# sunshinnnn/DSMnet

Hardware: AMD Instinct MI355X
Metric: stereo pairs/sec forward, PSMNet D=192 384×1280, at 1/2/4/8 MI355X (higher is better)
Workload: dtype f32

## Files before the change

dsmnet_amd/_lib.py:

```python
import ctypes
import os

_HERE = os.path.dirname(os.path.abspath(__file__))
LIB_PATH = os.environ.get("DSM_LIB_PATH") or os.path.join(_HERE, "csrc", "libdsmnet_hip.so")

c_int, c_void_p, c_size_t = ctypes.c_int, ctypes.c_void_p, ctypes.c_size_t

DSM_OK = 0
DSM_F32 = 0
DSM_NCDHW, DSM_NDHWC = 0, 1
DSM_CONV_FP32_MFMA, DSM_CONV_COUT1_CHUNKED, DSM_CONV_TM_SHIFT, DSM_CONV_BLOCKS_SHIFT = 1, 2, 4, 16
DSM_CONV_NO_NSPLIT = 4
DSM_CONV_NO_ONCE = 8
DSM_CONV_KSPLIT_SHIFT = 8
DSM_PREC_F32, DSM_PREC_F16, DSM_PREC_F16X2 = 0, 1, 2


class Bn3dArgs(ctypes.Structure):
    _fields_ = [("y", c_void_p), ("residual", c_void_p), ("out", c_void_p), ("gamma", c_void_p),
                ("beta", c_void_p), ("running_mean", c_void_p), ("running_var", c_void_p),
                ("affine", c_void_p), ("workspace", c_void_p), ("gout", c_void_p), ("dy", c_void_p),
                ("dresidual", c_void_p), ("B", c_int), ("C", c_int),
                ("Dy", c_int), ("Hy", c_int), ("Wy", c_int), ("Dr", c_int), ("Hr", c_int), ("Wr", c_int),
                ("relu", c_int), ("momentum", ctypes.c_float), ("eps", ctypes.c_float),
# ... 42 lines not shown
class ColorRecord(ctypes.Structure):
    _fields_ = [("order", c_int * 4), ("jitter", ctypes.c_float * 4), ("flags", c_int), ("alpha_row", c_int)]


DSM_COLOR_JITTER, DSM_COLOR_LIGHTING, DSM_COLOR_NORMALIZE = 1, 2, 4
DSM_COLOR_MAX_RECORDS = 64


SIGNATURES = {
    "dsm_abi_version": (c_int, []),
    "dsm_strerror": (ctypes.c_char_p, [c_int]),
    "dsm_corr1d_fwd": (c_int, [c_void_p] * 4 + [c_int] * 8 + [c_void_p]),
    "dsm_corr1d_bwd": (c_int, [c_void_p] * 6 + [c_int] * 8 + [c_void_p]),
    "dsm_concat_volume_fwd": (c_int, [c_void_p] * 3 + [c_int] * 8 + [c_void_p]),
    "dsm_concat_volume_bwd": (c_int, [c_void_p] * 3 + [c_int] * 8 + [c_void_p]),
    "dsm_soft_argmin_fwd": (c_int, [c_void_p] * 3 + [c_int] * 10 + [c_void_p]),
    "dsm_soft_argmin_bwd": (c_int, [c_void_p] * 5 + [c_int] * 10 + [c_void_p]),
    "dsm_corr1d_plan": (c_int, [c_void_p] * 4 + [c_int] * 8 + [ctypes.c_char_p, c_int]),
    "dsm_concat_volume_fwd_plan": (c_int, [c_void_p] * 3 + [c_int] * 8 + [ctypes.c_char_p, c_int]),
    "dsm_concat_volume_bwd_plan": (c_int, [c_void_p] * 3 + [c_int] * 8 + [ctypes.c_char_p, c_int]),
    "dsm_soft_argmin_fwd_plan": (c_int, [c_void_p] * 3 + [c_int] * 10 + [ctypes.c_char_p, c_int]),
    "dsm_soft_argmin_bwd_plan": (c_int, [c_void_p] * 5 + [c_int] * 10 + [ctypes.c_char_p, c_int]),
    "dsm_conv3d_packed_weight_bytes": (c_size_t, [c_int] * 3),
    "dsm_conv3d_pack_weights": (c_int, [c_void_p] * 2 + [c_int] * 3 + [c_void_p]),
    "dsm_conv_pack_weights": (c_int, [c_void_p] * 2 + [c_int] * 5 + [c_void_p]),
    "dsm_absmax": (c_int, [c_void_p, c_size_t, c_void_p, c_void_p]),
    "dsm_conv3d_fwd": (c_int, [ctypes.POINTER(Conv3dArgs), c_void_p]),
    "dsm_basicblock2d_fwd": (c_int, [ctypes.POINTER(BasicBlock2dArgs), c_void_p]),
    "dsm_conv3d_plan": (c_int, [ctypes.POINTER(Conv3dArgs), ctypes.c_char_p, c_int]),
    "dsm_conv3d_workspace_bytes": (c_size_t, [ctypes.POINTER(Conv3dArgs)]),
    "dsm_conv3d_wgrad": (c_int, [c_void_p] * 4 + [c_int] * 12 + [c_void_p] * 3),
    "dsm_conv2d_wgrad": (c_int, [c_void_p] * 4 + [c_int] * 11 + [c_void_p] * 3),
    "dsm_conv3d_cout1_bwd": (c_int, [c_void_p] * 5 + [c_int] * 5 + [c_void_p]),
    "dsm_deconv3d_cout1_bwd": (c_int, [c_void_p] * 5 + [c_int] * 8 + [c_void_p]),
    "dsm_bn3d_train_fwd": (c_int, [ctypes.POINTER(Bn3dArgs), c_void_p]),
    "dsm_bn3d_train_bwd": (c_int, [ctypes.POINTER(Bn3dArgs), c_void_p]),
    "dsm_decoder_cat": (c_int, [c_void_p] * 5 + [c_int] * 11 + [c_void_p]),
    "dsm_stage_images_nhwc16": (c_int, [c_void_p] * 3 + [c_int] * 4 + [c_void_p]),
    "dsm_volume_relayout": (c_int, [c_void_p] * 2 + [c_int] * 6 + [c_void_p]),
    "dsm_conv_packed_weight_bytes": (ctypes.c_size_t, [c_int] * 4),
    "dsm_spp_branch_floats": (ctypes.c_size_t, [c_int] * 3),
    "dsm_spp_pool8": (c_int, [c_void_p] * 2 + [c_int] * 3 + [c_void_p]),
    "dsm_spp_branches": (c_int, [c_void_p] * 5 + [c_int] * 3 + [c_void_p]),
    "dsm_spp_concat": (c_int, [c_void_p] * 4 + [c_int] * 3 + [c_void_p] * 2),
    "dsm_warp_abs_error": (c_int, [c_void_p] * 4 + [c_int] * 6 + [ctypes.c_float, c_void_p]),
    "dsm_selfsup_workspace_floats": (c_size_t, [ctypes.POINTER(SelfsupItem), c_int]),
    "dsm_selfsup_fwd": (c_int, [ctypes.POINTER(SelfsupItem), c_int, c_int] + [c_void_p] * 4),
    "dsm_selfsup_bwd": (c_int, [ctypes.POINTER(SelfsupItem), c_int, c_int] + [c_void_p] * 4),
    "dsm_suploss_workspace_floats": (c_size_t, [c_int] * 5),
    "dsm_suploss_fwd": (c_int, [ctypes.POINTER(SuplossItem), c_int, c_void_p, c_int, c_int, c_int, c_int] + [c_void_p] * 4),
    "dsm_suploss_bwd": (c_int, [ctypes.POINTER(SuplossItem), c_int, c_void_p, c_int, c_int, c_int] + [c_void_p] * 4),
    "dsm_stereo_color": (c_int, [c_void_p, c_void_p, ctypes.POINTER(ColorRecord)] + [c_int] * 6 + [c_void_p]),
    "dsm_concat_conv_fwd": (c_int, [c_void_p] * 5 + [c_size_t] + [c_void_p] * 2 + [c_int] * 9 + [c_void_p]),
}

_lib = None


class DsmnetHipError(RuntimeError):
    pass


def _bind_torch_hip_runtime():
    import torch
    hip = os.path.join(os.path.dirname(torch.__file__), "lib", "libamdhip64.so")
    if os.path.exists(hip):
        ctypes.CDLL(hip, mode=ctypes.RTLD_GLOBAL)


def load():
    global _lib
    if _lib is not None:
        return _lib
    if not os.path.exists(LIB_PATH):
        raise DsmnetHipError(
            "libdsmnet_hip.so not found at %s -- build it with "
            "`python -m dsmnet_amd.csrc.build` (there is no CPU fallback)" % LIB_PATH)
    _bind_torch_hip_runtime()
    lib = ctypes.CDLL(LIB_PATH)
    for name, (res, args) in SIGNATURES.items():
        fn = getattr(lib, name)
        fn.restype = res
        fn.argtypes = args
    if lib.dsm_abi_version() != 7:
        raise DsmnetHipError("libdsmnet_hip.so ABI version mismatch")
    _lib = lib
    return lib


def check(code, what):
    if code != DSM_OK:
        msg = load().dsm_strerror(code).decode()
        raise DsmnetHipError("%s failed: %s (code %d)" % (what, msg, code))
```

dsmnet_amd/blocks2d.py:

```python
import torch
import torch.nn as nn
import torch.nn.functional as F

from . import costvolume as cv
from . import blocks3d
from .blocks3d import _versions

_TRAIN_2D_MODE = __import__("os").environ.get("DSM_TRAIN_2D", "auto")
_FUSED_TRAIN_2D = _TRAIN_2D_MODE in ("auto", "fused", "conv")
_FUSED_TRAIN_2D_BN = _TRAIN_2D_MODE == "fused"
_TRAIN_2D_MIN_PIXELS = int(__import__("os").environ.get("DSM_TRAIN_2D_MIN_PIXELS", 65536)) if _TRAIN_2D_MODE == "auto" else 0


class own_kernels_only(object):

    def __enter__(self):
        global _TRAIN_2D_MIN_PIXELS, _FUSED_TRAIN_2D
        self.saved = (_TRAIN_2D_MIN_PIXELS, _FUSED_TRAIN_2D)
        _TRAIN_2D_MIN_PIXELS, _FUSED_TRAIN_2D = 0, True
        return self

    def __exit__(self, *exc):
        global _TRAIN_2D_MIN_PIXELS, _FUSED_TRAIN_2D
        _TRAIN_2D_MIN_PIXELS, _FUSED_TRAIN_2D = self.saved
        return False


def fused_ok(conv, x):
    if not (isinstance(conv, nn.Conv2d) and x.is_cuda and x.dtype == torch.float32):
        return False
    k, s, d, p = conv.kernel_size, conv.stride, conv.dilation, conv.padding
    if k[0] != k[1] or s[0] != s[1] or d[0] != d[1] or p[0] != p[1] or conv.groups != 1:
        return False
    if k[0] not in (1, 3) or s[0] not in (1, 2) or d[0] not in (1, 2):
        return False
    if p[0] != d[0] * (k[0] - 1) // 2 or conv.padding_mode != "zeros":
        return False
    if conv.out_channels in cv.WIDE2D_COUT:
        return _wide_ok(conv, x)
    if conv.out_channels not in (32, 64, 128):
        return False
    cin = x.shape[1]
    if cin % 16 != 0 or cin < conv.in_channels:
        return False
    return cv.conv2d_variant(conv.out_channels, s[0], k[0], d[0])


_WIDE2D_EXCLUDED = frozenset()


def _wide_ok(conv, x):
    if conv.kernel_size[0] != 3 or conv.dilation[0] != 1 or cv.get_option("conv_precision") not in ("f16x2", "f16"):
        return False
    B, cin, H, W = x.shape
    s = conv.stride[0]
    if cin % 16 != 0 or cin != conv.in_channels or (cin, conv.out_channels, s) in _WIDE2D_EXCLUDED:
        return False
    Ho, Wo = (H - 1) // s + 1, (W - 1) // s + 1
    if Wo > (2032 if s == 1 else 1016) or B * Ho * Wo >= 2 ** 20:
        return False
    return 4 * B * cin * H * W < 2 ** 31 and B * Ho * Wo * conv.out_channels < 2 ** 31 - 1


class _Folded2d(object):
    def __init__(self):
        self.key = None
        self.packed = self.scale = self.shift = None

    def get(self, conv, bn, cin_padded):
        srcs = [conv.weight, conv.bias]
        if bn is not None:
            srcs += [bn.weight, bn.bias, bn.running_mean, bn.running_var]
        key = _versions(*srcs) + (cin_padded,)
        if key != self.key:
            with torch.no_grad():
                self.packed = cv.pack_conv2d_weight(conv.weight, cin_padded)
                if bn is not None:
                    inv = torch.rsqrt(bn.running_var + bn.eps)
                    scale = bn.weight * inv if bn.weight is not None else inv
                    shift = -bn.running_mean * scale
                    if bn.bias is not None:
                        shift = shift + bn.bias
                    if conv.bias is not None:
                        shift = shift + conv.bias * scale
                    self.scale, self.shift = scale.contiguous(), shift.contiguous()
                elif conv.bias is not None:
                    self.scale = torch.ones_like(conv.bias)
                    self.shift = conv.bias.detach().clone()
                else:
                    self.scale = self.shift = None
            self.key = key
        return self.packed, self.scale, self.shift


def train_ok(conv, x):
    if not (_FUSED_TRAIN_2D and isinstance(conv, nn.Conv2d) and torch.is_tensor(x) and x.is_cuda and
            x.dtype == torch.float32 and conv.weight.dtype == torch.float32):
        return False
    k, s, d, p = conv.kernel_size, conv.stride, conv.dilation, conv.padding
    if k[0] != k[1] or s[0] != s[1] or d[0] != d[1] or p[0] != p[1] or conv.groups != 1:
        return False
    if conv.bias is not None or conv.padding_mode != "zeros" or p[0] != d[0] * (k[0] // 2):
        return False
    if x.shape[0] * ((x.shape[2] - 1) // s[0] + 1) * ((x.shape[3] - 1) // s[0] + 1) < _TRAIN_2D_MIN_PIXELS:
        return False
    return x.shape[1] == conv.in_channels and cv.conv2d_variant(conv.out_channels, s[0], k[0], d[0])


def _run_conv2d_autograd(conv, bn, x, residual, relu):
    y = cv.conv2d(x, conv.weight, conv.stride[0], conv.dilation[0])
    if (bn is not None and bn.training and _FUSED_TRAIN_2D_BN and blocks3d._FUSED_TRAIN_BN and
            y.shape[1] % 4 == 0 and y.shape[1] <= 256):
        momentum = bn.momentum if bn.momentum is not None else 0.1
        out = cv.bn_add_relu2d(y, bn.weight, bn.bias, residual,
                               bn.running_mean if bn.track_running_stats else None,
                               bn.running_var if bn.track_running_stats else None,
                               1 if relu else 0, momentum, bn.eps)
        if bn.num_batches_tracked is not None:
            bn.num_batches_tracked += 1
        blocks3d._bump_running_stats(bn)
        return out
    if bn is not None:
        y = bn(y)
    if residual is not None:
        y = y + residual
    return F.relu(y) if relu else y


def run_conv2d(folded, conv, bn, x, residual=None, relu=False):
    training = bn is not None and bn.training
    if not training and not torch.is_grad_enabled() and fused_ok(conv, x):
        packed, scale, shift = folded.get(conv, bn, x.shape[1])
        return cv.conv2d_block(x, packed, conv.out_channels, scale, shift, residual,
                               stride=conv.stride[0], relu=1 if relu else 0,
                               k=conv.kernel_size[0], dilation=conv.dilation[0])
    if train_ok(conv, x):
        return _run_conv2d_autograd(conv, bn, x, residual, relu)
    if x.shape[1] != conv.in_channels:
        x = x[:, : conv.in_channels]
    y = conv(x)
    if bn is not None:
        y = bn(y)
    if residual is not None:
        y = y + residual
    return F.relu(y) if relu else y


def run_basicblock_layers(fold1, c1, b1, fold2, c2, b2, x, relu_after, skip=True):
    if b1 is None or b2 is None or c1.training or b1.training or b2.training or torch.is_grad_enabled():
        return None
    if not (fused_ok(c1, x) and fused_ok(c2, x) and c1.kernel_size[0] == 3 and c2.kernel_size[0] == 3 and
            c2.stride[0] == 1 and c2.dilation[0] == 1 and c2.in_channels == c2.out_channels == c1.out_channels and
            cv.basicblock2d_ok(x, c1.in_channels, c1.out_channels, c1.stride[0], c1.dilation[0])):
        return None
    p1, s1, h1 = fold1.get(c1, b1, x.shape[1])
    p2, s2, h2 = fold2.get(c2, b2, x.shape[1])
    return cv.basicblock2d(x, p1, s1, h1, p2, s2, h2, relu=relu_after, skip=skip)


def run_basicblock(cb1, cb2, x, downsample):
    if downsample is not None or not isinstance(cb1, ConvBN2d) or not isinstance(cb2, ConvBN2d):
        return None
    return run_basicblock_layers(cb1._folded, cb1[0], cb1[1], cb2._folded, cb2[0], cb2[1], x, False)


class ConvBN2d(nn.Sequential):

    def __init__(self, conv, bn):
        super(ConvBN2d, self).__init__(conv, bn)
        self._folded = _Folded2d()

    def forward(self, x, residual=None, relu=False):
        return run_conv2d(self._folded, self[0], self[1], x, residual, relu)


def stage_image_nhwc16(img):
    return cv.stage_images_nhwc16(img, None)
```

dsmnet_amd/costvolume.py:

```python
import ctypes

import torch

from . import _lib

_CL3D = torch.channels_last_3d


class LaunchTimer(object):

    def __init__(self):
        self.records = []

    def start(self):
        ev = torch.cuda.Event(enable_timing=True)
        ev.record()
        return ev

    def stop(self, name, start, work):
        ev = torch.cuda.Event(enable_timing=True)
        ev.record()
        self.records.append((name, start, ev, work))

    def summary(self):
# ... 313 lines not shown
    a.x = x.data_ptr()
    a.w_packed = packed_weight.data_ptr()
    a.y = y.data_ptr()
    a.scale = None if scale is None else scale.data_ptr()
    a.shift = None if shift is None else shift.data_ptr()
    a.residual = None if residual is None else residual.data_ptr()
    a.B, a.Cin, a.Cout = B, cin, cout
    a.Di, a.Hi, a.Wi = Di, Hi, Wi
    a.Do, a.Ho, a.Wo = Do, Ho, Wo
    a.stride, a.transposed, a.relu = int(stride), int(transposed), int(relu)
    a.flags = _conv_flags()
    if virtual is not None:
        a.vol_virtual, a.vol_mask_left = 1, int(virtual.mask_left)
    keep = _set_precision(a, x, y if cout > 1 else None)
    vox = B * (Di * Hi * Wi if transposed else Do * Ho * Wo)
    work = 54.0 * cin * cout * vox if cout > 1 else 4.0 * B * (cin * Di * Hi * Wi + Do * Ho * Wo)
    with torch.cuda.device(x.device), _timed(lambda: conv3d_plan_name(a), work):
        rc = _lib.load().dsm_conv3d_fwd(ctypes.byref(a), _stream())
    _lib.check(rc, "dsm_conv3d_fwd")
    del keep
    return y


def conv3d_plan_name(args):
    buf = ctypes.create_string_buffer(96)
    _lib.check(_lib.load().dsm_conv3d_plan(ctypes.byref(args), buf, 96), "dsm_conv3d_plan")
    return buf.value.decode()


import os as _os

_PRECISIONS = ("bf16x3", "fp32", "f16x2", "f16")


def _env_precision():
    v = _os.environ.get("DSM_CONV_PRECISION", "")
    if v and v not in _PRECISIONS:
        raise ValueError("DSM_CONV_PRECISION must be one of %s, got %r" % (_PRECISIONS, v))
    return v or "f16x2"


def _env_flag(name, default):
    v = _os.environ.get(name, "")
    if v not in ("", "0", "1"):
        raise ValueError("%s must be 0 or 1, got %r" % (name, v))
    return default if v == "" else v == "1"


_WIDE_CONV2D_DEFAULT = False

_OPTIONS = {"fuse_volume": True, "fuse_blocks": True, "conv_precision": _env_precision(), "conv_flags": 0,
            "separable_volume": _env_flag("DSM_SEPARABLE_VOLUME", True), "separable_flags": 0,
            "fused_supervised_loss": _env_flag("DSM_FUSED_SUP_LOSS", True),
            "wide_conv2d": _env_flag("DSM_WIDE_CONV2D", _WIDE_CONV2D_DEFAULT)}


def set_option(name, value):
    if name == "conv_fp32":
        old = _OPTIONS["conv_precision"] == "fp32"
        _OPTIONS["conv_precision"] = "fp32" if value else "bf16x3"
        return old
    if name not in _OPTIONS:
        raise KeyError(name)
    old = _OPTIONS[name]
    if name == "conv_precision":
        if value not in _PRECISIONS:
            raise ValueError("conv_precision must be one of %s" % (_PRECISIONS,))
        _OPTIONS[name] = value
    else:
        _OPTIONS[name] = int(value) if name in ("conv_flags", "separable_flags") else bool(value)
    return old


def _conv_flags():
    return (_lib.DSM_CONV_FP32_MFMA if _OPTIONS["conv_precision"] == "fp32" else 0) | _OPTIONS["conv_flags"]


def get_option(name):
    if name == "conv_fp32":
        return _OPTIONS["conv_precision"] == "fp32"
    return _OPTIONS[name]


class _AmaxArena(object):
    SLOTS = 2048

    def __init__(self):
        self.buf, self.used, self.depth = {}, {}, 0

    def begin(self, device):
        key = (device.type, device.index)
        if key not in self.buf:
            self.buf[key] = torch.zeros(self.SLOTS, device=device, dtype=torch.float32)
        else:
            self.buf[key].zero_()
        self.used[key] = 0

    def slot(self, device):
        key = (device.type, device.index)
        if self.depth > 0 and key in self.buf and self.used[key] < self.SLOTS:
            i = self.used[key]
            self.used[key] = i + 1
            return self.buf[key][i:i + 1]
        return torch.zeros(1, device=device, dtype=torch.float32)


_ARENA = _AmaxArena()
# ... 459 lines not shown
        relu, rshape, has_gamma, has_beta = ctx.cfg
        gout = gout.contiguous(memory_format=_CL3D)
        B, C, Dy, Hy, Wy = y.shape
        a = _lib.Bn3dArgs()
        a.B, a.C, a.Dy, a.Hy, a.Wy = B, C, Dy, Hy, Wy
        dy = torch.empty_like(y, memory_format=_CL3D)
        dres = None
        if rshape is not None:
            a.Dr, a.Hr, a.Wr = rshape[2:]
            if ctx.needs_input_grad[3]:
                dres = torch.empty(rshape, device=y.device, dtype=torch.float32, memory_format=_CL3D)
                a.dresidual = dres.data_ptr()
            else:
                a.residual = y.data_ptr()
        ws = torch.empty(2 * C, device=y.device, dtype=torch.float64)
        a.y, a.affine, a.workspace = y.data_ptr(), affine.data_ptr(), ws.data_ptr()
        a.out = None if out is None else out.data_ptr()
        a.gout, a.dy, a.relu = gout.data_ptr(), dy.data_ptr(), relu
        if needs_amax():
            dy._dsm_amax = _ARENA.slot(y.device)
            a.dy_amax = dy._dsm_amax.data_ptr()
            if dres is not None:
                dres._dsm_amax = _ARENA.slot(y.device)
                a.dres_amax = dres._dsm_amax.data_ptr()
        with torch.cuda.device(y.device), _timed("bn3d_train_bwd_kernels", 4.0 * (3 * y.numel() + gout.numel())):
            rc = _lib.load().dsm_bn3d_train_bwd(ctypes.byref(a), _stream())
        _lib.check(rc, "dsm_bn3d_train_bwd")
        dbeta = ws[:C].float() if has_beta else None
        dgamma = ws[C:].float() if has_gamma else None
        return dy, dgamma, dbeta, dres, None, None, None, None, None


def bn_add_relu3d(y, gamma, beta, residual, running_mean, running_var, relu, momentum, eps):
    return BnAddRelu3dFunction.apply(y, gamma, beta, residual, running_mean, running_var, int(relu),
                                     float(momentum), float(eps))


def stage_images_nhwc16(left, right=None):
    _require_device("stage_images_nhwc16", left, right)
    left = left.contiguous()
    B, C, H, W = left.shape
    if right is not None:
        if tuple(right.shape) != tuple(left.shape):
            raise ValueError("stage_images_nhwc16: the two views differ in shape")
        right = right.contiguous()
    out = torch.empty(((1 if right is None else 2) * B, 16, H, W), device=left.device,
                      dtype=torch.float32, memory_format=_CL2D)
    with torch.cuda.device(left.device):
        rc = _lib.load().dsm_stage_images_nhwc16(_p(left), _p(right), _p(out), B, C, H, W, _stream())
    _lib.check(rc, "dsm_stage_images_nhwc16")
    return out


_CONV2D_VARIANTS = {(1, 1, 3, 1), (1, 2, 3, 1), (1, 4, 3, 1), (1, 4, 3, 2), (2, 1, 3, 1),
                    (2, 2, 3, 1), (1, 1, 1, 1), (1, 4, 1, 1), (2, 2, 1, 1)}


def conv2d_variant(cout, stride, k, dilation):
    return cout in (32, 64, 128) and (stride, cout // 32, k, dilation) in _CONV2D_VARIANTS


def _wgrad2d(x_cl, g_cl, stride, dilation):
    B, cx, Hx, Wx = x_cl.shape
    _, cg, Hg, Wg = g_cl.shape
    ws = torch.empty((cx // 32) * (cg // 32) * 9 * 1024, device=x_cl.device, dtype=torch.float32)
    dw = torch.empty((cg, cx, 3, 3), device=x_cl.device, dtype=torch.float32)
    prec, xa, ga = _wgrad_precision(x_cl, g_cl)
    with torch.cuda.device(x_cl.device), _timed("conv2d_wgrad_kernel", 18.0 * cx * cg * B * Hg * Wg):
        rc = _lib.load().dsm_conv2d_wgrad(_p(x_cl), _p(g_cl), _p(ws), _p(dw), B, cx, cg, Hx, Wx,
                                          Hg, Wg, int(stride), int(dilation), _conv_flags(), prec,
                                          _p(xa), _p(ga), _stream())
    _lib.check(rc, "dsm_conv2d_wgrad")
    return dw


class Conv2dFunction(torch.autograd.Function):

    @staticmethod
    def forward(ctx, x, weight, stride, dilation):
        _require_device("Conv2dFunction", x, weight)
        cout, cin, k, _ = weight.shape
        x = x.contiguous(memory_format=_CL2D)
        xs = x
        if cin % 16:
            xs = torch.zeros((x.shape[0], (cin + 15) // 16 * 16) + tuple(x.shape[2:]), device=x.device,
                             dtype=x.dtype).contiguous(memory_format=_CL2D)
            xs[:, :cin] = x
        packed = pack_conv2d_weight(weight, xs.shape[1])
        y = conv2d_block(xs, packed, cout, stride=stride, k=k, dilation=dilation)
        ctx.save_for_backward(x, weight)
        ctx.cfg = (int(stride), int(dilation))
        return y

    @staticmethod
    def backward(ctx, gy):
        x, weight = ctx.saved_tensors
        stride, dil = ctx.cfg
        cout, cin, k, _ = weight.shape
        gy = gy.contiguous(memory_format=_CL2D)
        w = weight.detach()
        need_dx, need_dw = ctx.needs_input_grad[0], ctx.needs_input_grad[1]
        dx = dw = None
        if need_dx and stride == 1 and conv2d_variant(cin, 1, k, dil) and cout % 16 == 0:
            wt = (w.flip(2, 3) if k == 3 else w).transpose(0, 1).contiguous()
            dx = conv2d_block(gy, pack_conv2d_weight(wt), cin, stride=1, k=k, dilation=dil)
        if need_dw and k == 3 and cin % 32 == 0 and cout % 32 == 0:
# ... 300 lines not shown
```

dsmnet_amd/csrc/build.py:

```python
import os
import subprocess
import sys
from concurrent.futures import ThreadPoolExecutor

HERE = os.path.dirname(os.path.abspath(__file__))
SOURCES = ["abi.hip", "corr1d.hip", "cost_volume.hip", "soft_argmin.hip", "conv3d.hip", "conv_f16.hip",
           "conv3d_bwd.hip", "bn3d.hip", "decoder.hip", "spp.hip", "warp.hip",
           "selfsup.hip", "color.hip", "sepvol.hip", "suploss.hip"]
LIB = os.path.join(HERE, "libdsmnet_hip.so")
HIPCC = os.environ.get("HIPCC", "/opt/rocm/bin/hipcc")
FLAGS = ["--offload-arch=gfx950", "-O3", "-std=c++17", "-fPIC",
         "-Wall", "-Wno-unused-function"] + os.environ.get("HIPCC_EXTRA", "").split()


def _stale(out, deps):
    if not os.path.exists(out):
        return True
    t = os.path.getmtime(out)
    return any(os.path.getmtime(d) > t for d in deps)


def build(force=False, verbose=True, stamps=False):
    if stamps:
        lib = os.path.join(HERE, "libdsmnet_hip_stamps.so")
        srcs = [os.path.join(HERE, s) for s in SOURCES]
        extra = ["-DDSM_ABLATE=%s" % os.environ["DSM_ABLATE"]] if os.environ.get("DSM_ABLATE") else []
        cmd = [HIPCC] + FLAGS + ["-DDSM_STAMPS"] + extra + ["-shared", "-o", lib] + srcs
        print(" ".join(cmd), flush=True)
        subprocess.run(cmd, check=True)
        return lib
    hdrs = [os.path.join(HERE, "common.hpp"), os.path.join(HERE, "conv_split.hpp"), os.path.join(HERE, "conv_zs.hpp"), os.path.join(HERE, "deconv_zs.hpp"), os.path.join(HERE, "conv_common.hpp"),
            os.path.join(HERE, "basicblock2d.hpp"), os.path.join(HERE, "conv_wide2d.hpp"),
            os.path.join(HERE, "..", "..", "include", "dsmnet_hip.h")]
    srcs = [os.path.join(HERE, s) for s in SOURCES if os.path.exists(os.path.join(HERE, s))]
    objs = []
    jobs = []
    for s in srcs:
        o = s[:-4] + ".o"
        objs.append(o)
        if force or _stale(o, [s] + hdrs):
            jobs.append([HIPCC] + FLAGS + ["-c", s, "-o", o])

    def run(cmd):
        if verbose:
            print(" ".join(cmd), flush=True)
        r = subprocess.run(cmd, capture_output=True, text=True)
        if r.returncode != 0:
            raise RuntimeError("hipcc failed:\n%s\n%s" % (r.stdout, r.stderr))
        if verbose and r.stderr.strip():
            print(r.stderr)

    with ThreadPoolExecutor(max_workers=min(4, max(1, len(jobs)))) as ex:
        list(ex.map(run, jobs))
    if jobs or force or _stale(LIB, objs):
        run([HIPCC, "--offload-arch=gfx950", "-shared", "-fPIC", "-o", LIB] + objs)
    return LIB


if __name__ == "__main__":
    print(build(force="--force" in sys.argv, stamps="--stamps" in sys.argv))
```

dsmnet_amd/models/psmnet/stackhourglass.py:

```python
import math

import torch
import torch.nn as nn

from ... import costvolume as cv
from ...blocks3d import Chain3d, ConvBN3d
from .submodule import convbn_3d, disparityregression, feature_extraction


def myadd_3d(tensor1, tensor2):
    assert tensor1.dim() == 5
    d, h, w = (min(a, b) for a, b in zip(tensor1.shape[2:], tensor2.shape[2:]))
    return tensor1[:, :, :d, :h, :w] + tensor2[:, :, :d, :h, :w]


def _deconvbn_3d(cin, cout):
    return ConvBN3d(nn.ConvTranspose3d(cin, cout, kernel_size=3, padding=1, output_padding=1,
                                       stride=2, bias=False), nn.BatchNorm3d(cout))


class hourglass(nn.Module):
    def __init__(self, inplanes):
        super(hourglass, self).__init__()
        c = inplanes
        self.conv1 = Chain3d(convbn_3d(c, c * 2, kernel_size=3, stride=2, pad=1), nn.ReLU(inplace=True))
        self.conv2 = convbn_3d(c * 2, c * 2, kernel_size=3, stride=1, pad=1)
        self.conv3 = Chain3d(convbn_3d(c * 2, c * 2, kernel_size=3, stride=2, pad=1), nn.ReLU(inplace=True))
        self.conv4 = Chain3d(convbn_3d(c * 2, c * 2, kernel_size=3, stride=1, pad=1), nn.ReLU(inplace=True))
        self.conv5 = _deconvbn_3d(c * 2, c * 2)
        self.conv6 = _deconvbn_3d(c * 2, c)

    def forward(self, x, presqu, postsqu, skip=None):
        out = self.conv1(x)
        pre = self.conv2(out, residual=postsqu, relu=True)
        out = self.conv4(self.conv3(pre))
        post = self.conv5(out, residual=presqu if presqu is not None else pre, relu=True)
        return self.conv6(post, residual=skip), pre, post


class PSMNet(nn.Module):

    def __init__(self, maxdisp=192, align_corners=False):
        super(PSMNet, self).__init__()
        self.name = "psmnet"
        self.maxdisp = maxdisp
        self.align_corners = bool(align_corners)
        self.count_levels = 1
        self.feature_extraction = feature_extraction(align_corners=align_corners)
        relu = lambda: nn.ReLU(inplace=True)
        self.dres0 = Chain3d(convbn_3d(64, 32, 3, 1, 1), relu(), convbn_3d(32, 32, 3, 1, 1), relu())
        self.dres1 = Chain3d(convbn_3d(32, 32, 3, 1, 1), relu(), convbn_3d(32, 32, 3, 1, 1))
        self.dres2 = hourglass(32)
        self.dres3 = hourglass(32)
        self.dres4 = hourglass(32)
        for i in (1, 2, 3):
            setattr(self, "classif%d" % i, Chain3d(
                convbn_3d(32, 32, 3, 1, 1), relu(),
                nn.Conv3d(32, 1, kernel_size=3, padding=1, stride=1, bias=False)))
        self._init_weights()

    def _init_weights(self):
        for m in self.modules():
            if isinstance(m, (nn.Conv2d, nn.Conv3d)):
                fan = m.out_channels
                for k in m.kernel_size:
                    fan *= k
                m.weight.data.normal_(0, math.sqrt(2.0 / fan))
            elif isinstance(m, (nn.BatchNorm2d, nn.BatchNorm3d)):
                m.weight.data.fill_(1)
                m.bias.data.zero_()

    def features(self, left, right):
        if self.training:
            return self.feature_extraction(left), self.feature_extraction(right)
        fe = self.feature_extraction
        if left.is_cuda and not torch.is_grad_enabled() and left.shape[1] <= 16:
            both = fe(cv.stage_images_nhwc16(left, right), staged=True)
        else:
            both = self.feature_extraction(torch.cat([left, right], dim=0))
        self.__dict__["_both"] = both
        return (cv.carry_amax(both[: left.shape[0]], both), cv.carry_amax(both[left.shape[0]:], both))

    def regularise(self, cost):
        cost0 = self.dres0(cost)
        cost0 = self.dres1(cost0, residual=cost0)
        out1, pre1, post1 = self.dres2(cost0, None, None, skip=cost0)
        out2, pre2, post2 = self.dres3(out1, pre1, post1, skip=cost0)
        out3, pre3, post3 = self.dres4(out2, pre1, post2, skip=cost0)
        cost1 = self.classif1(out1)
        cost2 = self.classif2(out2, residual=cost1)
        cost3 = self.classif3(out3, residual=cost2)
        return cost1, cost2, cost3

    def forward(self, left, right, mode="train"):
        with cv.amax_scope(left.device):
            return self._forward(left, right)

    def _forward(self, left, right):
        self.__dict__["_both"] = None
        refimg_fea, targetimg_fea = self.features(left, right)
        both = self.__dict__.pop("_both")
        if (both is not None and cv.get_option("fuse_volume") and not torch.is_grad_enabled() and
                cv.virtual_volume_ok(both.shape[1])):
            cost = cv.VirtualVolume(both, self.maxdisp // 4, True)
        else:
            cost = cv.concat_volume(refimg_fea, targetimg_fea, self.maxdisp // 4, mask_left=True)
        size = (self.maxdisp, left.shape[2], left.shape[3])
        cost1, cost2, cost3 = self.regularise(cost)
        pred1 = cv.soft_argmin(cost1, size, align_corners=self.align_corners)
        pred2 = cv.soft_argmin(cost2, size, align_corners=self.align_corners)
        pred3 = cv.soft_argmin(cost3, size, align_corners=self.align_corners)
        return [0, 0, 0], [pred3, pred2, pred1]
```

dsmnet_amd/models/psmnet/submodule.py:

```python
import torch
import torch.nn as nn
import torch.nn.functional as F

from ... import blocks2d
from ... import costvolume as cv
from ...blocks2d import ConvBN2d, _Folded2d, run_conv2d, stage_image_nhwc16
from ...blocks3d import ConvBN3d, _versions

_SPP_MATMUL = __import__("os").environ.get("DSM_TRAIN_SPP", "matmul") != "interp"
_TRAIN_NHWC = __import__("os").environ.get("DSM_TRAIN_LAYOUT", "nchw") == "nhwc"


def convbn(in_planes, out_planes, kernel_size, stride, pad, dilation):
    del pad
    return ConvBN2d(
        nn.Conv2d(in_planes, out_planes, kernel_size=kernel_size, stride=stride,
                  padding=dilation, dilation=dilation, bias=False),
        nn.BatchNorm2d(out_planes))


def convbn_3d(in_planes, out_planes, kernel_size, stride, pad):
    conv = nn.Conv3d(in_planes, out_planes, kernel_size=kernel_size, padding=pad,
                     stride=stride, bias=False)
    return ConvBN3d(conv, nn.BatchNorm3d(out_planes))
# ... 65 lines not shown

    @staticmethod
    def _bilinear_matrix(n_in, n_out, align_corners, device):
        i = torch.arange(n_out, dtype=torch.float32, device=device)
        if align_corners:
            src = i * ((n_in - 1) / (n_out - 1)) if n_out > 1 else torch.zeros_like(i)
        else:
            src = ((i + 0.5) * (n_in / n_out) - 0.5).clamp_min(0.0)
        i0 = src.floor().long().clamp_max(n_in - 1)
        i1 = (i0 + 1).clamp_max(n_in - 1)
        w1 = src - i0.to(src.dtype)
        m = torch.zeros((n_out, n_in), dtype=torch.float32, device=device)
        m.scatter_add_(1, i0[:, None], (1.0 - w1)[:, None])
        m.scatter_add_(1, i1[:, None], w1[:, None])
        return m

    def _upsample(self, y, size):
        if not (y.is_cuda and torch.is_grad_enabled() and _SPP_MATMUL):
            return F.interpolate(y, size=size, mode="bilinear", align_corners=self.align_corners)
        key = (y.shape[2], y.shape[3], size[0], size[1], self.align_corners, y.device)
        cache = self.__dict__.setdefault("_up_cache", {})
        if key not in cache:
            cache[key] = (self._bilinear_matrix(y.shape[2], size[0], self.align_corners, y.device),
                          self._bilinear_matrix(y.shape[3], size[1], self.align_corners, y.device).t().contiguous())
        ry, rxt = cache[key]
        return torch.matmul(ry, torch.matmul(y.contiguous(), rxt))

    def _spp_stock(self, raw, skip):
        size = skip.shape[2:]
        pooled, pyramid = skip, []
        for i in (4, 3, 2, 1):
            pooled = F.avg_pool2d(pooled, 8 if i == 4 else 2)
            branch = getattr(self, "branch%d" % i)
            y = branch[1](pooled, relu=True)
            pyramid.append(self._upsample(y, size))
        return torch.cat([raw, skip] + pyramid, dim=1)

    def _spp_params(self):
        convs = [getattr(self, "branch%d" % i)[1] for i in (4, 3, 2, 1)]
        srcs = [t for c in convs for t in (c[0].weight, c[1].weight, c[1].bias,
                                           c[1].running_mean, c[1].running_var)]
        key = _versions(*srcs)
        if getattr(self, "_spp_key", None) != key:
            with torch.no_grad():
                w_t = torch.stack([c[0].weight.reshape(32, 128).t() for c in convs]).contiguous()
                inv = [torch.rsqrt(c[1].running_var + c[1].eps) for c in convs]
                scale = torch.stack([c[1].weight * i for c, i in zip(convs, inv)])
                shift = torch.stack([c[1].bias - c[1].running_mean * s
                                     for c, s in zip(convs, scale)])
            self._spp_cache = (w_t, scale.contiguous(), shift.contiguous())
            self._spp_key = key
        return self._spp_cache

    def forward(self, x, staged=False):
        fast = x.is_cuda and not self.training and not torch.is_grad_enabled()
        if staged and not fast:
            raise RuntimeError("feature_extraction: staged input exists on the eval fast path only")
        if fast and not staged:
            x = stage_image_nhwc16(x)
        elif _TRAIN_NHWC and x.is_cuda:
            x = x.contiguous(memory_format=torch.channels_last)
        x = self.firstconv[0](x, relu=True)
        fc2, fc4 = self.firstconv[2], self.firstconv[4]
        y = blocks2d.run_basicblock_layers(fc2._folded, fc2[0], fc2[1], fc4._folded, fc4[0], fc4[1], x, True, skip=False)
        x = y if y is not None else fc4(fc2(x, relu=True), relu=True)
        x = self.layer1(x)
        raw = self.layer2(x)
        skip = self.layer4(self.layer3(raw))
        if skip.is_cuda and not self.training and not torch.is_grad_enabled() and not self.align_corners:
            x = cv.spp_head(raw, skip, *self._spp_params())
        else:
            x = self._spp_stock(raw, skip)
        x = self.lastconv[0](x, relu=True)
        if not hasattr(self, "_last_fold"):
            self._last_fold = _Folded2d()
        return run_conv2d(self._last_fold, self.lastconv[2], None, x)
```

include/dsmnet_hip.h:

```cpp
#ifndef DSMNET_HIP_H
#define DSMNET_HIP_H

#include <stddef.h>
#include <stdint.h>

#ifdef __cplusplus
extern "C" {
#endif

#define DSM_ABI_VERSION 7

#define DSM_OK               0
#define DSM_ERR_ARG         -1
#define DSM_ERR_UNSUPPORTED -2
#define DSM_ERR_LAUNCH      -3
#define DSM_ERR_ALIGN       -4

enum dsm_dtype  { DSM_F32 = 0 };
enum dsm_layout { DSM_NCDHW = 0, DSM_NDHWC = 1 };

typedef void* dsm_stream_t;

int         dsm_abi_version(void);
const char* dsm_strerror(int code);
// ... 179 lines not shown
  const void* disp_other;
  void* grad_disp;
  void* grad_other;
  int im_stride[4];
  int src_stride[4];
  int B, h, w, H0, W0;
  int left, top, scale_factor;
  float delt_im, delt_disp, weight;
  int pad_;
} dsm_selfsup_item;

size_t dsm_selfsup_workspace_floats(const dsm_selfsup_item* items, int n_items);
int dsm_selfsup_fwd(const dsm_selfsup_item* items, int n_items, int flag_mask, void* workspace,
                    void* loss, void* aux, dsm_stream_t stream);
int dsm_selfsup_bwd(const dsm_selfsup_item* items, int n_items, int flag_mask, const void* workspace,
                    const void* aux, const void* grad_loss, dsm_stream_t stream);

#define DSM_SUPLOSS_MAX_ITEMS 16
typedef struct dsm_suploss_item {
  const void* pred;
  void* grad;
  int B, hc, wc, level;
  float weight;
  int pad_[3];
} dsm_suploss_item;

size_t dsm_suploss_workspace_floats(int n_items, int B, int H, int W, int save_for_bwd);
int dsm_suploss_fwd(const dsm_suploss_item* items, int n_items, const void* gt, int H, int W,
                    int flag_smooth, int save_for_bwd, void* workspace, void* loss, void* aux,
                    dsm_stream_t stream);
int dsm_suploss_bwd(const dsm_suploss_item* items, int n_items, const void* gt, int H, int W,
                    int flag_smooth, const void* workspace, const void* aux, const void* grad_loss,
                    dsm_stream_t stream);

#define DSM_COLOR_JITTER     1
#define DSM_COLOR_LIGHTING   2
#define DSM_COLOR_NORMALIZE  4
#define DSM_COLOR_MAX_RECORDS 64
typedef struct dsm_color_record {
  int order[4];
  float jitter[4];
  int flags;
  int alpha_row;
} dsm_color_record;

int dsm_stereo_color(void* x, const void* alpha, const dsm_color_record* recs, int n_recs, int B, int C,
                     int H, int W, int groups, dsm_stream_t stream);

int dsm_concat_conv_fwd(const void* both, const void* w_packed, const void* scale, const void* shift,
                        void* workspace, size_t workspace_floats, void* y, float* y_amax,
                        int B, int C, int Cout, int D, int H, int W,
                        int mask_left, int relu, int flags, dsm_stream_t stream);

#ifdef __cplusplus
}
#endif
#endif
```

Measured before the change: 209.0.

## Add direct stereo stem conv and MFMA pointwise 1x1 kernels for feature tower

Adds a stem kernel that reads both raw NCHW left and right images directly and computes the 3->32 stride-2 3x3 conv with folded BN and ReLU, writing channels-last output. This skips the separate NHWC16 staging and concat pass. Also adds an MFMA-based 1x1 pointwise conv kernel, used for downsample and last conv layers in eval mode. These kernels target the 2D feature extraction, which is a small share of the PSMNet forward pass, so the overall gain is likely limited.

```diff
diff --git a/dsmnet_amd/_lib.py b/dsmnet_amd/_lib.py
--- a/dsmnet_amd/_lib.py
+++ b/dsmnet_amd/_lib.py
@@ -118,6 +118,8 @@
     "dsm_suploss_bwd": (c_int, [ctypes.POINTER(SuplossItem), c_int, c_void_p, c_int, c_int, c_int] + [c_void_p] * 4),
     "dsm_stereo_color": (c_int, [c_void_p, c_void_p, ctypes.POINTER(ColorRecord)] + [c_int] * 6 + [c_void_p]),
     "dsm_concat_conv_fwd": (c_int, [c_void_p] * 5 + [c_size_t] + [c_void_p] * 2 + [c_int] * 9 + [c_void_p]),
+    "dsm_stem2d_fwd": (c_int, [c_void_p] * 7 + [c_int] * 5 + [c_void_p]),
+    "dsm_pointwise2d_fwd": (c_int, [c_void_p] * 6 + [c_int] * 7 + [c_void_p]),
 }
 
 _lib = None
diff --git a/dsmnet_amd/blocks2d.py b/dsmnet_amd/blocks2d.py
--- a/dsmnet_amd/blocks2d.py
+++ b/dsmnet_amd/blocks2d.py
@@ -67,14 +67,14 @@
         self.key = None
         self.packed = self.scale = self.shift = None
 
-    def get(self, conv, bn, cin_padded):
+    def get(self, conv, bn, cin_padded, pack=True):
         srcs = [conv.weight, conv.bias]
         if bn is not None:
             srcs += [bn.weight, bn.bias, bn.running_mean, bn.running_var]
-        key = _versions(*srcs) + (cin_padded,)
+        key = _versions(*srcs) + (cin_padded, pack)
         if key != self.key:
             with torch.no_grad():
-                self.packed = cv.pack_conv2d_weight(conv.weight, cin_padded)
+                self.packed = cv.pack_conv2d_weight(conv.weight, cin_padded) if pack else conv.weight.detach().contiguous()
                 if bn is not None:
                     inv = torch.rsqrt(bn.running_var + bn.eps)
                     scale = bn.weight * inv if bn.weight is not None else inv
@@ -127,8 +127,29 @@
     return F.relu(y) if relu else y
 
 
-def run_conv2d(folded, conv, bn, x, residual=None, relu=False):
+def seam_ok(conv, x, residual=None):
+    return (residual is None and isinstance(conv, nn.Conv2d) and conv.kernel_size == (1, 1) and
+            conv.padding == (0, 0) and conv.groups == 1 and conv.bias is None and conv.stride[0] == conv.stride[1] and
+            cv.pointwise2d_ok(x, conv.in_channels, conv.out_channels, conv.stride[0]))
+
+
+def stem_ok(conv, x):
+    return (isinstance(conv, nn.Conv2d) and (conv.in_channels, conv.out_channels) == (3, 32) and
+            conv.kernel_size == (3, 3) and conv.stride == (2, 2) and conv.padding == (1, 1) and
+            conv.dilation == (1, 1) and conv.groups == 1 and conv.bias is None and conv.padding_mode == "zeros" and
+            not torch.is_grad_enabled() and cv.stem2d_ok(x))
+
+
+def run_stem(cb, left, right=None):
+    w, scale, shift = cb._folded.get(cb[0], cb[1], 3, pack=False)
+    return cv.stem2d(left, right, w, scale, shift)
+
+
+def run_conv2d(folded, conv, bn, x, residual=None, relu=False, seam=False):
     training = bn is not None and bn.training
+    if seam and not training and not torch.is_grad_enabled() and seam_ok(conv, x, residual):
+        w, scale, shift = folded.get(conv, bn, x.shape[1], pack=False)
+        return cv.pointwise2d(x, w, scale, shift, stride=conv.stride[0], relu=relu)
     if not training and not torch.is_grad_enabled() and fused_ok(conv, x):
         packed, scale, shift = folded.get(conv, bn, x.shape[1])
         return cv.conv2d_block(x, packed, conv.out_channels, scale, shift, residual,
@@ -171,7 +192,7 @@
         self._folded = _Folded2d()
 
     def forward(self, x, residual=None, relu=False):
-        return run_conv2d(self._folded, self[0], self[1], x, residual, relu)
+        return run_conv2d(self._folded, self[0], self[1], x, residual, relu, seam=True)
 
 
 def stage_image_nhwc16(img):
diff --git a/dsmnet_amd/costvolume.py b/dsmnet_amd/costvolume.py
--- a/dsmnet_amd/costvolume.py
+++ b/dsmnet_amd/costvolume.py
@@ -389,7 +389,8 @@
 _OPTIONS = {"fuse_volume": True, "fuse_blocks": True, "conv_precision": _env_precision(), "conv_flags": 0,
             "separable_volume": _env_flag("DSM_SEPARABLE_VOLUME", True), "separable_flags": 0,
             "fused_supervised_loss": _env_flag("DSM_FUSED_SUP_LOSS", True),
-            "wide_conv2d": _env_flag("DSM_WIDE_CONV2D", _WIDE_CONV2D_DEFAULT)}
+            "wide_conv2d": _env_flag("DSM_WIDE_CONV2D", _WIDE_CONV2D_DEFAULT),
+            "tower_seams": _env_flag("DSM_TOWER_SEAMS", True)}
 
 
 def set_option(name, value):
@@ -955,6 +956,71 @@
     return out
 
 
+def _seam_out(shape, device):
+    y = torch.empty(shape, device=device, dtype=torch.float32, memory_format=_CL2D)
+    ya = _ARENA.slot(device) if needs_amax() else None
+    if ya is not None:
+        y._dsm_amax = ya
+    return y, ya
+
+
+def stem2d_ok(left):
+    if not (_OPTIONS["tower_seams"] and torch.is_tensor(left) and left.is_cuda and left.dtype == torch.float32 and
+            left.dim() == 4 and left.shape[1] == 3):
+        return False
+    B, _, H, W = left.shape
+    return B * 3 * H * W < 2 ** 31 and 2 * B * ((H - 1) // 2 + 1) * ((W - 1) // 2 + 1) * 32 < 2 ** 31 and 2 * B <= 65535
+
+
+def stem2d(left, right, weight, scale=None, shift=None):
+    _require_device("stem2d", left, right, weight, scale, shift)
+    left = left.contiguous()
+    B, C, H, W = left.shape
+    if right is not None:
+        if tuple(right.shape) != tuple(left.shape):
+            raise ValueError("stem2d: the two views differ in shape")
+        right = right.contiguous()
+    weight = weight.detach().contiguous()
+    cout = weight.shape[0]
+    if tuple(weight.shape[1:]) != (C, 3, 3):
+        raise ValueError("stem2d: weight %s does not fit %d input channels, k3" % (tuple(weight.shape), C))
+    nB, Ho, Wo = (1 if right is None else 2) * B, (H - 1) // 2 + 1, (W - 1) // 2 + 1
+    y, ya = _seam_out((nB, cout, Ho, Wo), left.device)
+    work = 4.0 * (nB * C * H * W + y.numel())
+    with torch.cuda.device(left.device), _timed("conv2d_stem_kernel", work):
+        rc = _lib.load().dsm_stem2d_fwd(_p(left), _p(right), _p(weight), _p(scale), _p(shift), _p(y), _p(ya),
+                                        B, C, H, W, cout, _stream())
+    _lib.check(rc, "dsm_stem2d_fwd")
+    return y
+
+
+def pointwise2d_ok(x, cin, cout, stride):
+    if not (_OPTIONS["tower_seams"] and x.is_cuda and x.dtype == torch.float32 and x.dim() == 4 and
+            x.shape[1] == cin and cin in (32, 64, 128) and cout in (32, 64, 128) and stride in (1, 2)):
+        return False
+    B, _, H, W = x.shape
+    return x.numel() < 2 ** 31 and B * ((H - 1) // stride + 1) * ((W - 1) // stride + 1) * cout < 2 ** 31
+
+
+def pointwise2d(x, weight, scale=None, shift=None, stride=1, relu=False):
+    _require_device("pointwise2d", x, weight, scale, shift)
+    if not x.is_contiguous(memory_format=_CL2D):
+        x = carry_amax(x.contiguous(memory_format=_CL2D), x)
+    B, cin, H, W = x.shape
+    weight = weight.detach().contiguous()
+    cout = weight.shape[0]
+    if weight.numel() != cout * cin:
+        raise ValueError("pointwise2d: weight %s does not fit %d input channels, k1" % (tuple(weight.shape), cin))
+    Ho, Wo = (H - 1) // stride + 1, (W - 1) // stride + 1
+    y, ya = _seam_out((B, cout, Ho, Wo), x.device)
+    work = 4.0 * (B * Ho * Wo * cin + y.numel())
+    with torch.cuda.device(x.device), _timed("conv2d_pointwise_kernel<%d,%d,S=%d>" % (cin, cout, stride), work):
+        rc = _lib.load().dsm_pointwise2d_fwd(_p(x), _p(weight), _p(scale), _p(shift), _p(y), _p(ya),
+                                             B, cin, cout, H, W, int(stride), 1 if relu else 0, _stream())
+    _lib.check(rc, "dsm_pointwise2d_fwd")
+    return y
+
+
 _CONV2D_VARIANTS = {(1, 1, 3, 1), (1, 2, 3, 1), (1, 4, 3, 1), (1, 4, 3, 2), (2, 1, 3, 1),
                     (2, 2, 3, 1), (1, 1, 1, 1), (1, 4, 1, 1), (2, 2, 1, 1)}
 
diff --git a/dsmnet_amd/csrc/build.py b/dsmnet_amd/csrc/build.py
--- a/dsmnet_amd/csrc/build.py
+++ b/dsmnet_amd/csrc/build.py
@@ -6,7 +6,7 @@
 HERE = os.path.dirname(os.path.abspath(__file__))
 SOURCES = ["abi.hip", "corr1d.hip", "cost_volume.hip", "soft_argmin.hip", "conv3d.hip", "conv_f16.hip",
            "conv3d_bwd.hip", "bn3d.hip", "decoder.hip", "spp.hip", "warp.hip",
-           "selfsup.hip", "color.hip", "sepvol.hip", "suploss.hip"]
+           "selfsup.hip", "color.hip", "sepvol.hip", "suploss.hip", "tower_seams.hip"]
 LIB = os.path.join(HERE, "libdsmnet_hip.so")
 HIPCC = os.environ.get("HIPCC", "/opt/rocm/bin/hipcc")
 FLAGS = ["--offload-arch=gfx950", "-O3", "-std=c++17", "-fPIC",
diff --git a/dsmnet_amd/csrc/tower_seams.hip b/dsmnet_amd/csrc/tower_seams.hip
--- /dev/null
+++ b/dsmnet_amd/csrc/tower_seams.hip
@@ -0,0 +1,196 @@
+#include "common.hpp"
+
+namespace {
+
+__device__ __forceinline__ void wave_amax(float am, float* __restrict__ y_amax) {
+#pragma unroll
+  for (int o = 32; o; o >>= 1) am = fmaxf(am, __shfl_xor(am, o));
+  if ((threadIdx.x & 63) == 0 && am > __builtin_nontemporal_load(y_amax))
+    atomicMax(reinterpret_cast<unsigned*>(y_amax), __builtin_bit_cast(unsigned, am));
+}
+
+__device__ __forceinline__ float quad_amax(const f32x4 v) {
+  return fmaxf(fmaxf(fabsf(v.x), fabsf(v.y)), fmaxf(fabsf(v.z), fabsf(v.w)));
+}
+
+constexpr int ST_X = 32, ST_Y = 8, ST_PW = 2 * ST_X + 1, ST_PH = 2 * ST_Y + 1;
+constexpr int ST_PATCH = 3 * ST_PH * ST_PW, ST_LOADS = (ST_PATCH + 255) / 256;
+
+__global__ __launch_bounds__(256) void stem_kernel(const float* __restrict__ left, const float* __restrict__ right,
+                                                   const float* __restrict__ w, const float* __restrict__ scale,
+                                                   const float* __restrict__ shift, float* __restrict__ y,
+                                                   float* __restrict__ y_amax, int B, int H, int W, int Ho, int Wo) {
+  __shared__ float patch[ST_PATCH];
+  __shared__ f32x4 wl[27 * 8];
+  const int t = threadIdx.x;
+  const int n = blockIdx.z, oy0 = blockIdx.y * ST_Y, ox0 = blockIdx.x * ST_X;
+  const float* img = n < B ? left + (long)n * 3 * H * W : right + (long)(n - B) * 3 * H * W;
+  const int iy0 = 2 * oy0 - 1, ix0 = 2 * ox0 - 1;
+  float v[ST_LOADS];
+#pragma unroll
+  for (int i = 0; i < ST_LOADS; ++i) {
+    const int e = t + 256 * i;
+    const int px = e % ST_PW, r = e / ST_PW, py = r % ST_PH, c = r / ST_PH;
+    const int iy = iy0 + py, ix = ix0 + px;
+    const bool in = e < ST_PATCH && iy >= 0 && iy < H && ix >= 0 && ix < W;
+    v[i] = in ? img[((long)c * H + iy) * W + ix] : 0.f;
+  }
+  if (t < 27 * 8) {
+    const int tap = t >> 3, cq = t & 7;
+    wl[t] = f32x4{w[(4 * cq) * 27 + tap], w[(4 * cq + 1) * 27 + tap], w[(4 * cq + 2) * 27 + tap],
+                  w[(4 * cq + 3) * 27 + tap]};
+  }
+#pragma unroll
+  for (int i = 0; i < ST_LOADS; ++i)
+    if (t + 256 * i < ST_PATCH) patch[t + 256 * i] = v[i];
+  __syncthreads();
+
+  const int cq = t & 7, col = t >> 3;
+  f32x4 wr[27];
+#pragma unroll
+  for (int k = 0; k < 27; ++k) wr[k] = wl[k * 8 + cq];
+  const f32x4 sc = scale ? reinterpret_cast<const f32x4*>(scale)[cq] : f32x4{1.f, 1.f, 1.f, 1.f};
+  const f32x4 sh = shift ? reinterpret_cast<const f32x4*>(shift)[cq] : f32x4{0.f, 0.f, 0.f, 0.f};
+  const int ox = ox0 + col;
+  float am = 0.f;
+#pragma unroll 2
+  for (int row = 0; row < ST_Y; ++row) {
+    const int oy = oy0 + row;
+    f32x4 a = {0.f, 0.f, 0.f, 0.f};
+#pragma unroll
+    for (int c = 0; c < 3; ++c)
+#pragma unroll
+      for (int ky = 0; ky < 3; ++ky)
+#pragma unroll
+        for (int kx = 0; kx < 3; ++kx) {
+          const float xv = patch[(c * ST_PH + 2 * row + ky) * ST_PW + 2 * col + kx];
+          const f32x4 wv = wr[c * 9 + ky * 3 + kx];
+          a.x = fmaf(xv, wv.x, a.x); a.y = fmaf(xv, wv.y, a.y);
+          a.z = fmaf(xv, wv.z, a.z); a.w = fmaf(xv, wv.w, a.w);
+        }
+    f32x4 o;
+    o.x = fmaxf(fmaf(a.x, sc.x, sh.x), 0.f); o.y = fmaxf(fmaf(a.y, sc.y, sh.y), 0.f);
+    o.z = fmaxf(fmaf(a.z, sc.z, sh.z), 0.f); o.w = fmaxf(fmaf(a.w, sc.w, sh.w), 0.f);
+    if (oy < Ho && ox < Wo) {
+      reinterpret_cast<f32x4*>(y + (((long)n * Ho + oy) * Wo + ox) * 32)[cq] = o;
+      am = fmaxf(am, quad_amax(o));
+    }
+  }
+  if (y_amax) wave_amax(am, y_amax);
+}
+
+constexpr int PW_THREADS = 128, PW_PIX = 64;
+
+template <int CIN, int COUT>
+__global__ __launch_bounds__(PW_THREADS) void pointwise_kernel(const float* __restrict__ x, const float* __restrict__ w,
+                                                               const float* __restrict__ scale,
+                                                               const float* __restrict__ shift, float* __restrict__ y,
+                                                               float* __restrict__ y_amax, int npix, int Hi, int Wi,
+                                                               int Ho, int Wo, int stride, int relu) {
+  constexpr int NB = COUT / 32, NQ = CIN / 4, NM = CIN / 8;
+  __shared__ f32x4 wl[NB * NQ * 32];
+  const int lane = threadIdx.x & 63, p = lane & 31, h = lane >> 5;
+  const int pix = blockIdx.x * PW_PIX + (threadIdx.x >> 6) * 32 + p;
+  const bool valid = pix < npix;
+  const int pc = valid ? pix : 0;
+  const int xo = pc % Wo, yo = (pc / Wo) % Ho, b = pc / (Wo * Ho);
+  const f32x4* src = reinterpret_cast<const f32x4*>(x + (((long)b * Hi + yo * stride) * Wi + xo * stride) * CIN) + h;
+  f32x4 xv[NM];
+#pragma unroll
+  for (int m = 0; m < NM; ++m) xv[m] = src[2 * m];
+  for (int i = threadIdx.x; i < NB * NQ * 32; i += PW_THREADS) {
+    const int r = i & 31, q = (i >> 5) % NQ, nb = i / (32 * NQ);
+    wl[i] = reinterpret_cast<const f32x4*>(w)[(nb * 32 + r) * NQ + q];
+  }
+  __syncthreads();
+  f32x16 acc[NB];
+#pragma unroll
+  for (int nb = 0; nb < NB; ++nb)
+#pragma unroll
+    for (int k = 0; k < 16; ++k) acc[nb][k] = 0.f;
+#pragma unroll
+  for (int m = 0; m < NM; ++m) {
+    f32x4 wv[NB];
+#pragma unroll
+    for (int nb = 0; nb < NB; ++nb) wv[nb] = wl[(nb * NQ + 2 * m + h) * 32 + p];
+#pragma unroll
+    for (int j = 0; j < 4; ++j)
+#pragma unroll
+      for (int nb = 0; nb < NB; ++nb)
+        acc[nb] = __builtin_amdgcn_mfma_f32_32x32x2f32(wv[nb][j], xv[m][j], acc[nb], 0, 0, 0);
+  }
+  float am = 0.f;
+  f32x4* dst = reinterpret_cast<f32x4*>(y + (long)pc * COUT) + h;
+#pragma unroll
+  for (int nb = 0; nb < NB; ++nb)
+#pragma unroll
+    for (int g = 0; g < 4; ++g) {
+      const int cq = 8 * nb + 2 * g + h;
+      f32x4 o = {acc[nb][4 * g], acc[nb][4 * g + 1], acc[nb][4 * g + 2], acc[nb][4 * g + 3]};
+      if (scale) {
+        const f32x4 sc = reinterpret_cast<const f32x4*>(scale)[cq];
+        o.x *= sc.x; o.y *= sc.y; o.z *= sc.z; o.w *= sc.w;
+      }
+      if (shift) {
+        const f32x4 sh = reinterpret_cast<const f32x4*>(shift)[cq];
+        o.x += sh.x; o.y += sh.y; o.z += sh.z; o.w += sh.w;
+      }
+      if (relu) { o.x = fmaxf(o.x, 0.f); o.y = fmaxf(o.y, 0.f); o.z = fmaxf(o.z, 0.f); o.w = fmaxf(o.w, 0.f); }
+      if (valid) {
+        dst[8 * nb + 2 * g] = o;
+        am = fmaxf(am, quad_amax(o));
+      }
+    }
+  if (y_amax) wave_amax(am, y_amax);
+}
+
+template <int CIN, int COUT>
+int launch_pointwise(const void* x, const void* w, const void* scale, const void* shift, void* y, float* y_amax,
+                     long npix, int Hi, int Wi, int Ho, int Wo, int stride, int relu, hipStream_t stream) {
+  dsm_clear_stale_error();
+  hipLaunchKernelGGL((pointwise_kernel<CIN, COUT>), dim3((unsigned)((npix + PW_PIX - 1) / PW_PIX)), dim3(PW_THREADS), 0,
+                     stream, (const float*)x, (const float*)w, (const float*)scale, (const float*)shift, (float*)y,
+                     y_amax, (int)npix, Hi, Wi, Ho, Wo, stride, relu);
+  return dsm_launch_status();
+}
+
+}
+
+extern "C" int dsm_stem2d_fwd(const void* left, const void* right, const void* w, const void* scale,
+                              const void* shift, void* y, float* y_amax, int B, int C, int H, int W, int Cout,
+                              dsm_stream_t stream) {
+  DSM_REQUIRE(left && w && y && B > 0 && C > 0 && H > 0 && W > 0 && Cout > 0, DSM_ERR_ARG);
+  DSM_REQUIRE(C == 3 && Cout == 32, DSM_ERR_UNSUPPORTED);
+  const int Ho = (H - 1) / 2 + 1, Wo = (W - 1) / 2 + 1;
+  const long nB = right ? 2L * B : B;
+  DSM_REQUIRE((long)B * 3 * H * W < (1L << 31) && nB * Ho * Wo * 32 < (1L << 31) && nB <= 65535 &&
+              dsm_cdiv(Ho, ST_Y) <= 65535, DSM_ERR_UNSUPPORTED);
+  DSM_REQUIRE(dsm_aligned16(y) && (!scale || dsm_aligned16(scale)) && (!shift || dsm_aligned16(shift)), DSM_ERR_ALIGN);
+  dsm_clear_stale_error();
+  hipLaunchKernelGGL(stem_kernel, dim3(dsm_cdiv(Wo, ST_X), dsm_cdiv(Ho, ST_Y), (unsigned)nB), dim3(256), 0,
+                     (hipStream_t)stream, (const float*)left, (const float*)right, (const float*)w,
+                     (const float*)scale, (const float*)shift, (float*)y, y_amax, B, H, W, Ho, Wo);
+  return dsm_launch_status();
+}
+
+extern "C" int dsm_pointwise2d_fwd(const void* x, const void* w, const void* scale, const void* shift, void* y,
+                                   float* y_amax, int B, int Cin, int Cout, int H, int W, int stride, int relu,
+                                   dsm_stream_t stream) {
+  DSM_REQUIRE(x && w && y && B > 0 && Cin > 0 && Cout > 0 && H > 0 && W > 0, DSM_ERR_ARG);
+  DSM_REQUIRE(stride == 1 || stride == 2, DSM_ERR_ARG);
+  DSM_REQUIRE((Cin == 32 || Cin == 64 || Cin == 128) && (Cout == 32 || Cout == 64 || Cout == 128), DSM_ERR_UNSUPPORTED);
+  const int Ho = (H - 1) / stride + 1, Wo = (W - 1) / stride + 1;
+  const long npix = (long)B * Ho * Wo;
+  DSM_REQUIRE((long)B * H * W * Cin < (1L << 31) && npix * Cout < (1L << 31), DSM_ERR_UNSUPPORTED);
+  DSM_REQUIRE(dsm_aligned16(x) && dsm_aligned16(w) && dsm_aligned16(y) && (!scale || dsm_aligned16(scale)) &&
+              (!shift || dsm_aligned16(shift)), DSM_ERR_ALIGN);
+  const hipStream_t s = (hipStream_t)stream;
+#define DSM_PW(CI, CO) \
+  if (Cin == CI && Cout == CO) \
+    return launch_pointwise<CI, CO>(x, w, scale, shift, y, y_amax, npix, H, W, Ho, Wo, stride, relu, s);
+  DSM_PW(32, 32) DSM_PW(32, 64) DSM_PW(32, 128)
+  DSM_PW(64, 32) DSM_PW(64, 64) DSM_PW(64, 128)
+  DSM_PW(128, 32) DSM_PW(128, 64) DSM_PW(128, 128)
+#undef DSM_PW
+  return DSM_ERR_UNSUPPORTED;
+}
diff --git a/dsmnet_amd/models/psmnet/stackhourglass.py b/dsmnet_amd/models/psmnet/stackhourglass.py
--- a/dsmnet_amd/models/psmnet/stackhourglass.py
+++ b/dsmnet_amd/models/psmnet/stackhourglass.py
@@ -74,7 +74,9 @@
         if self.training:
             return self.feature_extraction(left), self.feature_extraction(right)
         fe = self.feature_extraction
-        if left.is_cuda and not torch.is_grad_enabled() and left.shape[1] <= 16:
+        if left.is_cuda and not torch.is_grad_enabled() and left.shape == right.shape and fe.stem_direct(left):
+            both = fe(left, right=right)
+        elif left.is_cuda and not torch.is_grad_enabled() and left.shape[1] <= 16:
             both = fe(cv.stage_images_nhwc16(left, right), staged=True)
         else:
             both = self.feature_extraction(torch.cat([left, right], dim=0))
diff --git a/dsmnet_amd/models/psmnet/submodule.py b/dsmnet_amd/models/psmnet/submodule.py
--- a/dsmnet_amd/models/psmnet/submodule.py
+++ b/dsmnet_amd/models/psmnet/submodule.py
@@ -141,15 +141,25 @@
             self._spp_key = key
         return self._spp_cache
 
-    def forward(self, x, staged=False):
+    def stem_direct(self, x):
+        return (x.is_cuda and not self.training and not self.firstconv[0][1].training and
+                blocks2d.stem_ok(self.firstconv[0][0], x))
+
+    def forward(self, x, staged=False, right=None):
         fast = x.is_cuda and not self.training and not torch.is_grad_enabled()
         if staged and not fast:
             raise RuntimeError("feature_extraction: staged input exists on the eval fast path only")
-        if fast and not staged:
-            x = stage_image_nhwc16(x)
-        elif _TRAIN_NHWC and x.is_cuda:
-            x = x.contiguous(memory_format=torch.channels_last)
-        x = self.firstconv[0](x, relu=True)
+        direct = fast and not staged and self.stem_direct(x)
+        if right is not None and not direct:
+            raise RuntimeError("feature_extraction: a second view exists on the direct-stem path only")
+        if direct:
+            x = blocks2d.run_stem(self.firstconv[0], x, right)
+        else:
+            if fast and not staged:
+                x = stage_image_nhwc16(x)
+            elif _TRAIN_NHWC and x.is_cuda:
+                x = x.contiguous(memory_format=torch.channels_last)
+            x = self.firstconv[0](x, relu=True)
         fc2, fc4 = self.firstconv[2], self.firstconv[4]
         y = blocks2d.run_basicblock_layers(fc2._folded, fc2[0], fc2[1], fc4._folded, fc4[0], fc4[1], x, True, skip=False)
         x = y if y is not None else fc4(fc2(x, relu=True), relu=True)
@@ -163,4 +173,4 @@
         x = self.lastconv[0](x, relu=True)
         if not hasattr(self, "_last_fold"):
             self._last_fold = _Folded2d()
-        return run_conv2d(self._last_fold, self.lastconv[2], None, x)
+        return run_conv2d(self._last_fold, self.lastconv[2], None, x, seam=not self.training)
diff --git a/include/dsmnet_hip.h b/include/dsmnet_hip.h
--- a/include/dsmnet_hip.h
+++ b/include/dsmnet_hip.h
@@ -255,6 +255,13 @@
                         int B, int C, int Cout, int D, int H, int W,
                         int mask_left, int relu, int flags, dsm_stream_t stream);
 
+int dsm_stem2d_fwd(const void* left, const void* right, const void* w, const void* scale,
+                   const void* shift, void* y, float* y_amax, int B, int C, int H, int W, int Cout,
+                   dsm_stream_t stream);
+int dsm_pointwise2d_fwd(const void* x, const void* w, const void* scale, const void* shift, void* y,
+                        float* y_amax, int B, int Cin, int Cout, int H, int W, int stride, int relu,
+                        dsm_stream_t stream);
+
 #ifdef __cplusplus
 }
 #endif
```

New measurement: 208.7. About the same (-0.2%).
